# wuxiaolang/Cube_SLAM_wu

Hardware: AMD Instinct MI355X
Metric: frames/sec detect_cuboid (higher is better)
Workload: dtype f64

## Files before the change

cube_slam_wu_amd/capi.py:

```python
from __future__ import annotations

import os as _os
_os.environ.setdefault("GPU_MAX_HW_QUEUES", "8")
import ctypes as C
import os

import numpy as np

_HERE = os.path.dirname(os.path.abspath(__file__))
LIB_PATH = os.path.join(_HERE, "libcubeslam_hip.so")


class CsDetectParams(C.Structure):
    _fields_ = [
        ("consider_config_1", C.c_int), ("consider_config_2", C.c_int),
        ("whether_sample_cam_roll_pitch", C.c_int), ("whether_sample_bbox_height", C.c_int),
        ("max_cuboid_num", C.c_int), ("nominal_skew_ratio", C.c_double), ("max_cut_skew", C.c_double),
        ("yaw_range_deg", C.c_double), ("yaw_step_deg", C.c_double),
        ("vp12_edge_angle_thre", C.c_double), ("vp3_edge_angle_thre", C.c_double), ("shorted_edge_thre", C.c_double),
        ("weight_vp_angle", C.c_double), ("weight_skew_error", C.c_double),
        ("pre_merge_dist_thre", C.c_double), ("pre_merge_angle_thre", C.c_double), ("edge_length_threshold", C.c_double),
        ("host_threads", C.c_int),
    ]

# ... 21 lines not shown
    ]


class CsDetectTiming(C.Structure):
    _fields_ = [(n, C.c_double) for n in ("setup_host_ms", "h2d_ms", "vp_kernel_ms", "cand_kernel_ms", "compact_ms", "d2h_ms",
                                          "rank_host_ms", "finalize_ms", "total_ms")] + \
               [("n_jobs", C.c_longlong), ("n_slots", C.c_longlong), ("n_valid", C.c_longlong),
                ("cand_kernel_bytes", C.c_longlong), ("cand_kernel_launches", C.c_int), ("n_fallback_boxes", C.c_int), ("n_redo_frames", C.c_int),
                ("rank_kernel_ms", C.c_double), ("line_setup_ms", C.c_double), ("score_kernel_ms", C.c_double), ("score_kernel_bytes", C.c_longlong)]


DECLARED_SYMBOLS = [
    "cs_last_error", "cs_device_count", "cs_diag_build", "cs_detect_default_params", "cs_box_rois", "cs_cam_euler_zyx", "cs_detector_create",
    "cs_detector_destroy", "cs_detect_cuboids", "cs_batch_create", "cs_batch_max_boxes", "cs_batch_run", "cs_batch_submit", "cs_batch_collect",
    "cs_bgr_to_gray", "cs_edge_distance_maps", "cs_edge_distance_maps_multi", "cs_detect_cuboids_gray", "cs_batch_create_gray", "cs_batch_refill_gray", "cs_batch_refill_wait", "cs_batch_destroy", "cs_batch_last_timing", "cs_batch_debug_candidates", "cs_batch_debug_kept", "cs_batch_set_debug", "cs_batch_set_pipeline_chunks", "cs_detect_lines_gray", "cs_detect_lines_batch", "cs_detect_lines_last_timing", "cs_detect_lsd_gray", "cs_detect_lsd_batch", "cs_detect_lsd_last_timing",
    "cs_check_score_atan2", "cs_check_score_sample_index",
]

_lib = None


def lib():
    global _lib
    if _lib is None:
        if not os.path.exists(LIB_PATH):
            raise RuntimeError("libcubeslam_hip.so not built: run `python -c 'import __graft_entry__ as g; g.build()'`")
        try:
            import torch
        except ImportError:
            pass
        L = C.CDLL(LIB_PATH)
# ... 307 lines not shown
            if rc < 0:
                raise RuntimeError("cs_batch_debug_candidates failed (%d): %s" % (rc, last_error()))
        return rows, corners

    def debug_kept(self, frame, box, k=0):
        L = lib()
        n = L.cs_batch_debug_kept(self.h, frame, box, k, 0, None, None)
        if n < 0:
            raise RuntimeError("cs_batch_debug_kept failed (%d)" % n)
        ids = np.zeros(n, np.int32)
        sc = np.zeros(n)
        if n:
            L.cs_batch_debug_kept(self.h, frame, box, k, n, ids.ctypes.data_as(C.POINTER(C.c_int)), _dp(sc))
        return ids, sc

    def close(self):
        if self.h:
            lib().cs_batch_destroy(self.h)
            self.h = C.c_void_p()

    def __del__(self):
        try:
            self.close()
        except Exception:
            pass


class CsBaTiming(C.Structure):
    _fields_ = [(n, C.c_double) for n in ("errors_ms", "linearize_ms", "reduce_ms", "schur_ms", "factor_ms", "backsub_ms", "update_ms", "total_ms")] + \
               [("n_linearizations", C.c_longlong), ("n_solves", C.c_longlong), ("linearize_bytes", C.c_longlong), ("schur_entries", C.c_longlong), ("structure_ms", C.c_double)]
# ... 655 lines not shown
```

cube_slam_wu_amd/csrc/detect_host.cpp:

```cpp
#include <hip/hip_runtime.h>

#include <algorithm>
#include <atomic>
#include <condition_variable>
#include <memory>
#include <mutex>
#include <chrono>
#include <cmath>
#include <limits>
#include <cstdio>
#include <cstring>
#include <functional>
#include <numeric>
#include <string>
#include <thread>
#include <vector>

#include "../../include/cubeslam_hip.h"
#include "cs_hip_util.h"
#include "detect_hooks.h"
#include "detect_types.h"
#include "edge_types.h"

thread_local std::string g_cs_err;
// ... 369 lines not shown
  std::vector<int> rp_idx;
  std::vector<int> keep;
  std::vector<double> score;
  std::vector<double> corners;
};

struct PipeSlot {
  DevBuf<cs::JobDesc> jobs;
  DevBuf<unsigned char> tab_arena;
  PinBuf<unsigned char> h_tab_arena;
  bool merged_io = false;
  size_t o_jobs = 0, o_rec = 0, o_wc = 0, o_fb = 0, o_jv = 0, o_cb = 0, o_end = 0;
  DevBuf<long long> slot_prefix, job_cbase, c_slot, fb_slot;
  DevBuf<int> vp_prefix, top_x, flag, job_valid, c_flag, box_job0, box_njobs, win_count, fallback, fb_flag;
  DevBuf<double> bound3;
  DevBuf<int> ls_order, blk_info, ls_crowded;
  PinBuf<int> h_ls_order;
  DevBuf<double> mid_x, mid_y, ang, yaw, yaw_c, yaw_s, vp, bound, c_dist, c_angle, c_skew, fb_dist, fb_angle, fb_skew;
  DevBuf<cs::RankWinner> winners;
  DevBuf<cs_cuboid> records;
  PinBuf<cs_cuboid> h_records;
  struct RpRound { size_t j0 = 0, nj = 0, b0 = 0, nb = 0; long long slot_cap = 0; int vp_cap = 0; };
  std::vector<RpRound> rp_rounds;
  std::vector<int> rp_box_frame, rp_box_index;
  DevBuf<int> rp_trip_cnt;
  DevBuf<int> rp_cur_idx, rp_tab_count, rp_maps;
  DevBuf<long long> rp_last_slot, rp_box_base;
  DevBuf<unsigned long long> rp_pool_used;
  DevBuf<double> rp_raw_euler;
  PinBuf<int> h_rp_tab_count, h_rp_maps;
// ... 10 lines not shown
  PinBuf<double> h_yaw, h_yaw_c, h_yaw_s;
  PinBuf<long long> h_fb_src, h_fb_dst, h_fb_slot, h_win_slots;
  PinBuf<int> h_fb_cnt, h_fb_flag;
  PinBuf<double> h_fb_dist, h_fb_angle, h_fb_skew, h_win_corners;
  hipEvent_t done = nullptr, ev[13] = {};
  cs::DetectDeviceView view{};
  int f0 = 0, f1 = 0, vp_total = 0;
  size_t nj = 0, nb = 0;
  long long slot_total = 0;
  bool in_flight = false;
  bool counted_busy = false;
  void release() {
    jobs.release(); slot_prefix.release(); job_cbase.release(); c_slot.release(); fb_slot.release();
    vp_prefix.release(); top_x.release(); flag.release(); job_valid.release(); c_flag.release(); box_job0.release(); box_njobs.release(); win_count.release();
    fallback.release(); fb_flag.release(); mid_x.release(); mid_y.release(); ang.release(); yaw.release(); yaw_c.release(); yaw_s.release();
    vp.release(); bound.release(); bound3.release(); ls_order.release(); blk_info.release(); ls_crowded.release(); h_ls_order.release(); c_dist.release(); c_angle.release(); c_skew.release(); fb_dist.release(); fb_angle.release(); fb_skew.release();
    winners.release(); records.release(); h_records.release(); rp_trip_cnt.release(); rp_cur_idx.release(); rp_tab_count.release(); rp_maps.release(); rp_last_slot.release(); rp_box_base.release(); rp_pool_used.release(); rp_raw_euler.release(); h_rp_tab_count.release(); h_rp_maps.release(); h_rp_raw_euler.release(); h_rp_last_slot.release(); h_rp_box_base.release(); h_rp_pool_used.release(); h_jobs_in.release(); h_jobs_out.release(); h_slot_prefix.release(); h_job_cbase.release(); h_vp_prefix.release();
    h_top_x.release(); h_box_job0.release(); h_box_njobs.release(); h_win_count.release(); h_fallback.release(); h_job_valid.release(); h_yaw.release();
    h_yaw_c.release(); h_yaw_s.release();
    h_fb_src.release(); h_fb_dst.release(); h_fb_slot.release(); h_win_slots.release(); h_fb_cnt.release(); h_fb_flag.release(); h_fb_dist.release(); h_fb_angle.release();
    h_fb_skew.release(); h_win_corners.release();
    if (done) (void)hipEventDestroy(done);
    for (auto& e : ev) if (e) (void)hipEventDestroy(e);
    for (auto& e : rp_ev) if (e) (void)hipEventDestroy(e);
    rp_ev.clear();
    done = nullptr; for (auto& e : ev) e = nullptr;
  }
};

struct BatchRunState;
struct cs_batch {
// ... 3 lines not shown
  DevBuf<unsigned char> d_gray, d_cls;
  DevBuf<cs::EdgeRoi> d_edge_rois;
  DevBuf<unsigned char> d_gray2;
  hipStream_t copy_stream = nullptr;
  hipEvent_t ev_copied[2] = {nullptr, nullptr}, ev_edge_done[2] = {nullptr, nullptr};
  int gray_cur = 0, gray_w = 0, gray_h = 0, edge_n_rois = 0, edge_max_w = 1;
  long long edge_max_px = 1;
  bool gray_batch = false;
  int refill_q[2] = {-1, -1}, n_refill = 0;
  PinBuf<float> h_maps_stage;
  PipeSlot pipe[2];
  std::vector<int> job_base, box_base, top_base;
  std::vector<long long> line_base;
  bool force_no_pipeline = false;
  int pipe_chunks = 1;
  int n_frames = 0, max_boxes = 0;
  std::vector<FrameIn> frames;
  DevBuf<float> d_maps;
  DevBuf<double> d_invK, d_frame_lines;
  DevBuf<int> d_frame_line_ptr;
  bool device_setup = false;
  bool force_host_setup = false;
  DevBuf<cs::JobDesc> d_jobs;
  DevBuf<long long> d_slot_prefix, d_job_cbase, d_c_slot, d_win_slots;
  DevBuf<int> d_vp_prefix, d_top_x, d_flag, d_job_valid, d_c_flag;
  DevBuf<double> d_mid_x, d_mid_y, d_ang, d_yaw, d_yaw_c, d_yaw_s, d_vp, d_bound, d_dist, d_angle, d_skew, d_corners, d_c_dist, d_c_angle, d_c_skew, d_win_corners;
  DevBuf<cs::RpPose> d_rp;
  PinBuf<char> h_stage;
  PinBuf<long long> h_c_slot, h_job_cbase;
  PinBuf<int> h_c_flag, h_job_valid;
// ... 653 lines not shown
      for (int q = 0; q < NBK; q++) cnt[q + 1] += cnt[q];
      for (size_t j = 0; j < nj; j++) S.h_ls_order.p[cnt[bucket(S.h_jobs_in.p[j])]++] = (int)j;
    }
    if (vo > 0x7fffffffLL) { cs_set_error("too many yaw samples in one chunk"); return CS_ERR_CAPACITY; }
  }
  S.nb = nb;
  MARK(1, tq);
  MARK(2, tq);
  C.tm->setup_host_ms += now_ms() - t0;
  C.tm->n_jobs += (long long)nj; C.tm->n_slots += real_slots;
  const long long slot_total = S.slot_total;
  PENS(S.ls_order, nj); PENS(S.jobs, nj); PENS(S.slot_prefix, nj + 1); PENS(S.vp_prefix, nj + 1); PENS(S.job_valid, nj); PENS(S.job_cbase, nj + 1);
  PENS(S.mid_x, n_lines + 1); PENS(S.mid_y, n_lines + 1); PENS(S.ang, n_lines + 1); PENS(S.yaw, n_yaw + 1); PENS(S.yaw_c, n_yaw + 1); PENS(S.yaw_s, n_yaw + 1);
  PENS(S.top_x, n_top + 1); PENS(S.vp, 6 * (size_t)S.vp_total + 6); PENS(S.bound, 6 * (size_t)S.vp_total + 6); PENS(S.bound3, nj * (size_t)cs::vp3_table_doubles_per_job());
  PENS(S.blk_info, 2 * (size_t)(slot_total >> 8) + 4); PENS(S.ls_crowded, 2 * (nj + 1) + 2);
  PENS(S.c_slot, slot_total + 1); PENS(S.c_flag, slot_total + 1); PENS(S.c_dist, slot_total + 1);
  PENS(S.c_angle, slot_total + 1); PENS(S.c_skew, slot_total + 1); PENS(S.box_job0, nb + 1); PENS(S.box_njobs, nb + 1); PENS(S.win_count, nb + 1);
  PENS(S.fallback, nb + 1); PENS(S.winners, nb * KMAX + 1); PENS(S.records, nb * KMAX + 1); PENS(S.h_records, nb * KMAX + 1);
  PENS(S.h_win_count, nb + 1); PENS(S.h_fallback, nb + 1); PENS(S.h_job_valid, nj); PENS(S.h_job_cbase, nj + 1); PENS(S.h_jobs_out, nj);
  int* p_ls_order = S.ls_order.p; cs::JobDesc* p_jobs = S.jobs.p; long long* p_slot_prefix = S.slot_prefix.p; int* p_vp_prefix = S.vp_prefix.p;
  double *p_yaw = S.yaw.p, *p_yaw_c = S.yaw_c.p, *p_yaw_s = S.yaw_s.p;
  int *p_top_x = S.top_x.p, *p_box_job0 = S.box_job0.p, *p_box_njobs = S.box_njobs.p;
  cs_cuboid* p_records = S.records.p; int *p_win_count = S.win_count.p, *p_fallback = S.fallback.p, *p_job_valid = S.job_valid.p; long long* p_job_cbase = S.job_cbase.p;
  std::unique_lock<std::mutex> enqueue(d->streams->enqueue_mu, std::defer_lock);
  S.merged_io = nj <= 256;
  if (S.merged_io) {
    size_t need = 0;
    auto room = [&](size_t bytes) { const size_t at = need; need += (bytes + 255) & ~(size_t)255; return at; };
    const size_t o_ls = room(sizeof(int) * nj), o_sp = room(sizeof(long long) * (nj + 1)), o_vp = room(sizeof(int) * (nj + 1));
    const size_t o_y = room(8 * n_yaw), o_yc = room(8 * n_yaw), o_ys = room(8 * n_yaw), o_tx = room(sizeof(int) * n_top), o_b0 = room(sizeof(int) * nb), o_bn = room(sizeof(int) * nb);
// ... 17 lines not shown
  } else {
    cs::CopySegs cp{};
    cs::add_copy(cp, S.ls_order, S.h_ls_order, nj); cs::add_copy(cp, S.jobs, S.h_jobs_in, nj); cs::add_copy(cp, S.slot_prefix, S.h_slot_prefix, nj + 1);
    cs::add_copy(cp, S.vp_prefix, S.h_vp_prefix, nj + 1); cs::add_copy(cp, S.yaw, S.h_yaw, n_yaw); cs::add_copy(cp, S.yaw_c, S.h_yaw_c, n_yaw);
    cs::add_copy(cp, S.yaw_s, S.h_yaw_s, n_yaw); cs::add_copy(cp, S.top_x, S.h_top_x, n_top); cs::add_copy(cp, S.box_job0, S.h_box_job0, nb);
    cs::add_copy(cp, S.box_njobs, S.h_box_njobs, nb);
    if (!d->streams->own_streams) enqueue.lock();
    cs::launch_multi_copy(cp, st);
  }
  cs::DetectDeviceView& v = S.view;
  v = cs::DetectDeviceView{};
  v.jobs = p_jobs; v.n_jobs = (int)nj; v.slot_prefix = p_slot_prefix; v.vp_prefix = p_vp_prefix; v.maps = b->d_maps.p;
  v.mid_x = S.mid_x.p; v.mid_y = S.mid_y.p; v.line_angle = S.ang.p; v.yaw = p_yaw; v.yaw_cos = p_yaw_c; v.yaw_sin = p_yaw_s; v.top_x = p_top_x;
  v.rp = b->d_rp.p; v.invK = b->d_invK.p; v.vp = S.vp.p; v.bound = S.bound.p; v.bound3 = S.bound3.p; v.job_valid = p_job_valid;
  v.job_cbase = p_job_cbase; v.c_slot = S.c_slot.p; v.c_flag = S.c_flag.p; v.c_dist = S.c_dist.p; v.c_angle = S.c_angle.p; v.c_skew = S.c_skew.p;
  hipStream_t stB = nullptr, stC = nullptr;
  sweep_side_streams(d, &stB, &stC);
  if (stB != st) {
    CS_HIP_TRY(hipEventRecord(S.ev[7], st));
    CS_HIP_TRY(hipStreamWaitEvent(stB, S.ev[7], 0));
  }
  CS_HIP_TRY(hipEventRecord(S.ev[8], stB));
  v.blk_info = S.blk_info.p;
  CS_HIP_TRY(hipMemsetAsync(S.blk_info.p, 0, sizeof(int), stB));
  cs::launch_candidate_compact(v, C.sp, stB);
  CS_HIP_TRY(hipEventRecord(S.ev[9], stB));
  CS_HIP_TRY(hipEventRecord(S.ev[10], stB));
  CS_HIP_TRY(hipEventRecord(S.ev[0], st));
  cs::launch_line_setup_listed(p_jobs, (int)nj, b->d_frame_lines.p, b->d_frame_line_ptr.p, S.mid_x.p, S.mid_y.p, S.ang.p, P.pre_merge_dist_thre, P.pre_merge_angle_thre, P.edge_length_threshold, st, p_ls_order,
                               stC, S.ev[0], S.ev[12], S.ls_crowded.p);
  CS_HIP_TRY(hipEventRecord(S.ev[1], st));
  cs::launch_vp_support_only(v, C.sp, S.vp_total, st, 1);
  CS_HIP_TRY(hipEventRecord(S.ev[2], st));
  if (stB != st) CS_HIP_TRY(hipStreamWaitEvent(st, S.ev[10], 0));
  CS_HIP_TRY(hipEventRecord(S.ev[4], st));
  cs::launch_score(v, C.sp, slot_total, slot_total, st);
  CS_HIP_TRY(hipEventRecord(S.ev[5], st));
  cs::RankView rv{};
  rv.box_job0 = p_box_job0; rv.box_njobs = p_box_njobs; rv.n_boxes = (int)nb; rv.winners = S.winners.p; rv.win_count = p_win_count; rv.fallback = p_fallback;
  cs::RankParams rkp{P.weight_vp_angle, P.weight_skew_error, P.nominal_skew_ratio, P.max_cut_skew, KMAX, C.sp.short_sq_bound};
  cs::launch_rank(v, rv, rkp, st, 0, false);
  cs::launch_records(v, rv, KMAX, p_records, st, nullptr, rkp.short_sq_bound);
  CS_HIP_TRY(hipEventRecord(S.ev[6], st));
  CS_HIP_TRY(hipGetLastError());
  if (S.merged_io) {
    CS_HIP_TRY(hipMemcpyAsync(S.h_tab_arena.p + S.o_jobs, S.tab_arena.p + S.o_jobs, S.o_end - S.o_jobs, hipMemcpyDeviceToHost, st));
  } else {
    cs::CopySegs cp{};
    cs::add_copy(cp, S.h_records, S.records, nb * KMAX); cs::add_copy(cp, S.h_win_count, S.win_count, nb); cs::add_copy(cp, S.h_fallback, S.fallback, nb);
// ... 580 lines not shown
  CS_GUARD_BEGIN
  return batch_run_impl(d, b, out, out_counts, false);
  CS_GUARD_END("cs_batch_run")
}
extern "C" int cs_batch_submit(cs_detector* d, cs_batch* b, cs_cuboid* out, int* out_counts) {
  CS_GUARD_BEGIN
  return batch_run_impl(d, b, out, out_counts, true);
  CS_GUARD_END("cs_batch_submit")
}
extern "C" int cs_batch_collect(cs_detector* d, cs_batch* b) {
  CS_GUARD_BEGIN
  if (!d || !b || b->det != d) return CS_ERR_INVALID_ARG;
  return batch_collect_impl(d, b);
  CS_GUARD_END("cs_batch_collect")
}
static void batch_drop_run_state(cs_batch* b) { delete b->run_state; b->run_state = nullptr; }
static int batch_collect_impl(cs_detector* d, cs_batch* b) {
  if (!b->run_state) return CS_OK;
  std::unique_ptr<BatchRunState> rs(b->run_state);
  b->run_state = nullptr;
  if (!rs->deferred) return CS_OK;
  CS_HIP_TRY(hipSetDevice(d->device));
  int rc = rs->rp_lean ? rp_finish(rs->C, b->pipe[0]) : pipe_finish(rs->C, b->pipe[0], rs->cam_rp);
  if (rc) return rc;
  rs->tm.total_ms = now_ms() - rs->t_begin;
  b->timing = rs->tm;
  b->ran = true;
  if (g_prof && (++g_runs % 8) == 0) {
    const char* nm[11] = {"jobs+samples", "prefix+pack", "box table", "alloc+enqueue", "gpu wait", "tie lists", "records", "tie wait", "tie rank", "tie corners", "tie records"};
    fprintf(stderr, "[detect] host ms/run:");
    for (int k = 0; k < 11; k++) { fprintf(stderr, " %s %.3f", nm[k], g_mark[k] / 8); g_mark[k] = 0; }
    fprintf(stderr, " | pre %.3f total %.3f\n", g_mark[11] / 8, rs->tm.total_ms); g_mark[11] = 0;
  }
  return CS_OK;
}
static int batch_run_impl(cs_detector* d, cs_batch* b, cs_cuboid* out, int* out_counts, bool defer) {
  if (!d || !b || b->det != d || !out || !out_counts) return CS_ERR_INVALID_ARG;
  if (b->run_state) { cs_set_error("cs_batch_submit: the previous submit of this batch has not been collected"); return CS_ERR_INVALID_ARG; }
  CS_HIP_TRY(hipSetDevice(d->device));
  { const int rcf = batch_flush_refill(d, b); if (rcf) return rcf; }
  std::unique_ptr<BatchRunState> rs_owner(new BatchRunState());
  BatchRunState* rs = rs_owner.get();
  const cs_detect_params& P = d->prm;
  const bool sample_rp = P.whether_sample_cam_roll_pitch != 0;
  const int NF = b->n_frames, MB = b->max_boxes, KMAX = P.max_cuboid_num;
  auto parallel_for = [d](int n, int , const std::function<void(int)>& fn) { d->pool->run(n, fn); };
  const int NT = d->n_threads;
  hipStream_t st = d->stream;
  cs_detect_timing& tm = rs->tm;
  double t_begin = now_ms();
  rs->t_begin = t_begin;

  std::fill(out_counts, out_counts + (size_t)NF * std::max(MB, 0), 0);
  b->results.clear();
  b->job_index.assign((size_t)NF * std::max(MB, 1) * 3, -1);

  cs::SweepParams sp;
  sp.vp12_thre_rad = P.vp12_edge_angle_thre / 180.0 * CS_PI;
  sp.vp3_thre_rad = P.vp3_edge_angle_thre / 180.0 * CS_PI;
  sp.short_thre = P.shorted_edge_thre;
  sp.short_sq_bound = cs::sqrt_lt_bound(P.shorted_edge_thre);
  sp.consider_config_1 = P.consider_config_1; sp.consider_config_2 = P.consider_config_2;

  double t0 = now_ms();
  std::vector<CamCache>& cam_raw = rs->cam_raw; cam_raw.resize(NF);
  std::vector<std::vector<CamCache>>& cam_rp = rs->cam_rp; cam_rp.resize(NF);
  std::vector<double> cur_yaw(NF);
  parallel_for(NF, NT, [&](int f) {
    const FrameIn& F = b->frames[f];
    make_cam(F.K, F.R, F.t, cam_raw[f]);
    cur_yaw[f] = cam_raw[f].cam_yaw;
    if (sample_rp) {
      std::vector<double> rs, ps;
      linespace<double>(cam_raw[f].euler[0] - 6.0 / 180.0 * CS_PI, cam_raw[f].euler[0] + 6.0 / 180.0 * CS_PI, 3.0 / 180.0 * CS_PI, rs);
      linespace<double>(cam_raw[f].euler[1] - 6.0 / 180.0 * CS_PI, cam_raw[f].euler[1] + 6.0 / 180.0 * CS_PI, 3.0 / 180.0 * CS_PI, ps);
      for (double r : rs)
        for (double p : ps) {
// ... 715 lines not shown
```

cube_slam_wu_amd/csrc/detect_kernels.hip:

```cpp
#include <hip/hip_runtime.h>
#include "cs_hip_util.h"

#include <cstdio>
#include <cstdlib>
#include <cstring>

#include "../../include/cubeslam_hip.h"
#include "detect_types.h"
#include "cs_atan2_lean.h"

namespace cs {

__device__ __forceinline__ int wave_uniform_i32(int x) { return __builtin_amdgcn_readfirstlane(x); }
__device__ __forceinline__ long long wave_uniform_i64(long long x) {
  const unsigned lo = (unsigned)__builtin_amdgcn_readfirstlane((int)(unsigned)(x & 0xffffffffll)), hi = (unsigned)__builtin_amdgcn_readfirstlane((int)(x >> 32));
  return (long long)(((unsigned long long)hi << 32) | lo);
}
__device__ __forceinline__ double wave_uniform_f64(double x) {
  int lo, hi;
  asm("v_readfirstlane_b32 %0, %1" : "=s"(lo) : "v"(__double2loint(x)));
  asm("v_readfirstlane_b32 %0, %1" : "=s"(hi) : "v"(__double2hiint(x)));
  return __hiloint2double(hi, lo);
}
template <typename T>
// ... 169 lines not shown
  }
  const double NaN = __builtin_nan("");
#pragma unroll
  for (int k = 0; k < K; k++) {
    const double ang_hi = R[k].have ? la[R[k].i_hi] : NaN, ang_lo = R[k].have ? la[R[k].i_lo] : NaN;
    out[2 * k] = swapped[k] ? ang_lo : ang_hi;
    out[2 * k + 1] = swapped[k] ? ang_hi : ang_lo;
  }
}

enum { VP3_RPCAP = 32 };

template <int MODE, bool UNIFORM>
__device__ __forceinline__ void vp_support_body(const DetectDeviceView& v, const SweepParams& sp, const JobDesc& jd, int j, long long e, bool on, VpChunk* ch) {
  int rp = 0, y = 0;
  if (on) {
    int local = (int)e - jd.vp_off;
    on = local < jd.RP * jd.Y;
    rp = local / jd.Y; y = local - rp * jd.Y;
  }
  double vpx[3] = {0, 0, 0}, vpy[3] = {0, 0, 0};
  if (on) {
    const RpPose* pose = v.rp + jd.rp_off + rp;
    double cy = v.yaw_cos[jd.yaw_off + y], sy = v.yaw_sin[jd.yaw_off + y];
    const double* A = pose->KinvR;
    double d[3][3] = {{cy, sy, 0.0}, {-sy, cy, 0.0}, {0.0, 0.0, 1.0}};
#pragma unroll
    for (int k = 0; k < 3; k++) {
      double h0 = (A[0] * d[k][0] + A[1] * d[k][1]) + A[2] * d[k][2];
      double h1 = (A[3] * d[k][0] + A[4] * d[k][1]) + A[5] * d[k][2];
      double h2 = (A[6] * d[k][0] + A[7] * d[k][1]) + A[8] * d[k][2];
      vpx[k] = h0 / h2;
      vpy[k] = h1 / h2;
    }
    if (MODE == 0) {
      double* vout = v.vp + 6 * e;
      vout[0] = vpx[0]; vout[1] = vpy[0]; vout[2] = vpx[1]; vout[3] = vpy[1]; vout[4] = vpx[2]; vout[5] = vpy[2];
    }
  }
  const double* mx = v.mid_x + jd.line_off;
  const double* my = v.mid_y + jd.line_off;
  const double* la = v.line_angle + jd.line_off;
  double b6[6];
  const double thre[3] = {sp.vp12_thre_rad, sp.vp12_thre_rad, sp.vp3_thre_rad};
  const bool swapped[3] = {false, true, true};
  vp_support_multi<(MODE == 0 ? 3 : 2), UNIFORM>(mx, my, la, jd.m, ch, vpx, vpy, thre, swapped, on, b6);
  if (!on) return;
  if (MODE == 1) { const double* t3 = v.bound3 + 2 * ((size_t)j * VP3_RPCAP + rp); b6[4] = t3[0]; b6[5] = t3[1]; }
  double* bout = v.bound + 6 * e;
#pragma unroll
  for (int q = 0; q < 6; q++) bout[q] = b6[q];
}

template <int MODE>
__global__ __launch_bounds__(256) void vp_support_kernel(DetectDeviceView v, SweepParams sp, int vp_total) {
  long long e = xcd_virtual_block() * blockDim.x + threadIdx.x;
  const bool on = e < vp_total;
  const int j = find_job_wave<int>(v.vp_prefix, v.n_jobs, on ? (int)e : vp_total - 1);
  const int ju = wave_uniform_i32(j);
  __shared__ VpChunk chunk[4];
  if (__all(j == ju)) vp_support_body<MODE, true>(v, sp, v.jobs[ju], ju, e, on, &chunk[threadIdx.x >> 6]);
  else vp_support_body<MODE, false>(v, sp, v.jobs[j], j, e, on, nullptr);
}
// ... 75 lines not shown
  unsigned long long valid = __ballot(flag != 0);
  if (valid) {
    int lane = threadIdx.x & 63;
    int j0 = __shfl(j, __ffsll((long long)valid) - 1);
    unsigned long long same = __ballot(flag != 0 && j == j0);
    if (same == valid) {
      if (lane == __ffsll((long long)valid) - 1) atomicAdd(&v.job_valid[j0], __popcll(valid));
    } else if (flag != 0) {
      atomicAdd(&v.job_valid[j], 1);
    }
  }
}

enum { COMPACT_PER = 16 };
enum { CC_TRIP = 4096 };
__global__ __launch_bounds__(256) void candidate_compact_kernel(DetectDeviceView v, SweepParams sp) {
  const int j = blockIdx.x;
  if (j >= v.n_jobs) return;
  __shared__ unsigned char s_flag[CC_TRIP];
  __shared__ int wsum[4];
  const int tid = threadIdx.x, lane = tid & 63, wid = tid >> 6;
  int jd_Y, jd_T, jd_rp_off, jd_yaw_off, jd_vp_off, jd_top_off, n_vp;
  BoxGeomD gd;
  {
    const JobDesc& jd = v.jobs[j];
    jd_Y = jd.Y; jd_T = jd.T; jd_rp_off = jd.rp_off; jd_yaw_off = jd.yaw_off; jd_vp_off = jd.vp_off; jd_top_off = jd.top_off;
    n_vp = jd.RP * jd.Y;
    const BoxGeomD g = box_geom_d(jd.g);
    gd = BoxGeomD{g.left, wave_uniform_f64(g.top), g.right, wave_uniform_f64(g.down),
                  wave_uniform_f64(g.el), wave_uniform_f64(g.et), wave_uniform_f64(g.er), wave_uniform_f64(g.eb)};
  }
  int* out_valid = v.job_valid + j;
  long long* out_cbase = v.job_cbase + j;
  asm volatile("" : "+v"(out_valid), "+v"(out_cbase));
  for (int e = tid; e < n_vp; e += 256) {
    const int rp = e / jd_Y, y = e - rp * jd_Y;
    const RpPose* pose = v.rp + jd_rp_off + rp;
    const double cy = v.yaw_cos[jd_yaw_off + y], sy = v.yaw_sin[jd_yaw_off + y];
    const double* A = pose->KinvR;
    const double d[3][3] = {{cy, sy, 0.0}, {-sy, cy, 0.0}, {0.0, 0.0, 1.0}};
    double* vout = v.vp + 6 * (long long)(jd_vp_off + e);
#pragma unroll
    for (int k = 0; k < 3; k++) {
      const double h0 = (A[0] * d[k][0] + A[1] * d[k][1]) + A[2] * d[k][2];
      const double h1 = (A[3] * d[k][0] + A[4] * d[k][1]) + A[5] * d[k][2];
      const double h2 = (A[6] * d[k][0] + A[7] * d[k][1]) + A[8] * d[k][2];
      vout[2 * k] = h0 / h2;
      vout[2 * k + 1] = h1 / h2;
    }
// ... 38 lines not shown
#pragma unroll
    for (int w = 0; w < 4; w++) { const int x = wsum[w]; if (w < wid) woff += x; total += x; }
    long long pos0 = run + woff;
    const long long sl0 = base + 2ll * r0 + wid * (64 * COMPACT_PER) + lane;
#pragma unroll
    for (int q = 0; q < COMPACT_PER; q++) {
      const unsigned long long bal = __ballot(f[q] != 0);
      if (f[q] != 0) {
        const long long pos = pos0 + __popcll(bal & below);
        v.c_slot[pos] = sl0 + q * 64;
        v.c_flag[pos] = f[q] | (j << CAND_JOB_SHIFT);
      }
      pos0 += __popcll(bal);
    }
    run += total;
    __syncthreads();
  }
  const int n_valid = (int)(run - base);
  if (tid == 0) { *out_valid = n_valid; *out_cbase = base; }
  const int nblk = (n_valid + 255) >> 8;
  if (nblk > 0) {
    __shared__ int s_at;
    if (tid == 0) s_at = atomicAdd(&v.blk_info[0], nblk);
    __syncthreads();
    const int at = s_at, b0 = (int)(base >> 8);
    for (int k = tid; k < nblk; k += 256) {
      const int left = n_valid - 256 * k;
      v.blk_info[2 + 2 * (long long)(at + k)] = b0 + k;
      v.blk_info[3 + 2 * (long long)(at + k)] = left > 256 ? 256 : left;
    }
  }
}

__device__ __forceinline__ int slot_corners(const DetectDeviceView& v, const JobDesc& jd, long long slot, double short_sq_bound, V2 c[8]) {
// ... 1208 lines not shown
    o.camera_pitch_delta = pose.pitch - raw_euler[3 * jd.frame + 1];
  }
  out[e] = o;
}

static inline unsigned grid8(long long n, int bs) {
  long long nb = (n + bs - 1) / bs;
  nb = (nb + 7) / 8 * 8;
  return (unsigned)(nb < 8 ? 8 : nb);
}

void launch_vp_support(const DetectDeviceView& v, const SweepParams& sp, int vp_total, hipStream_t st) {
  if (vp_total <= 0) return;
  vp_support_kernel<0><<<dim3(grid8(vp_total, 256)), dim3(256), 0, st>>>(v, sp, vp_total);
}
void launch_vp_support_only(const DetectDeviceView& v, const SweepParams& sp, int vp_total, hipStream_t st, int rp_max) {
  if (skip_kernel("vp_support")) return;
  if (vp_total <= 0) return;
  const int stride = (rp_max >= 1 && rp_max <= (int)VP3_RPCAP) ? rp_max : (int)VP3_RPCAP;
  hipLaunchKernelGGL(vp3_support_kernel, dim3((unsigned)(((long long)v.n_jobs * stride + 63) / 64)), dim3(64), 0, st, v, sp, stride);
  vp_support_kernel<1><<<dim3(grid8(vp_total, 256)), dim3(256), 0, st>>>(v, sp, vp_total);
}
int vp3_table_doubles_per_job() { return 2 * VP3_RPCAP; }
void launch_vp_points(const DetectDeviceView& v, int vp_total, hipStream_t st) {
  if (vp_total <= 0) return;
  hipLaunchKernelGGL(vp_points_kernel, dim3((vp_total + 255) / 256), dim3(256), 0, st, v, vp_total);
}
void launch_candidates(const DetectDeviceView& v, const SweepParams& sp, long long slot_total, hipStream_t st) {
  if (skip_kernel("candidate")) return;
  if (slot_total <= 0) return;
  hipLaunchKernelGGL(candidate_kernel, dim3(grid8(slot_total, 256)), dim3(256), 0, st, v, sp, slot_total);
}
void launch_candidate_compact(const DetectDeviceView& v, const SweepParams& sp, hipStream_t st) {
  if (skip_kernel("candidate")) return;
  if (v.n_jobs <= 0) return;
  hipLaunchKernelGGL(candidate_compact_kernel, dim3(v.n_jobs), dim3(256), 0, st, v, sp);
// ... 374 lines not shown
```

cube_slam_wu_amd/csrc/detect_types.h:

```cpp
#pragma once
#include <hip/hip_runtime.h>

#include <cstdint>

#include "../../include/cubeslam_hip.h"
#include "cs_geom.h"

namespace cs {

struct JobDesc {
  BoxGeom g;
  int map_w;
  int m;
  int Y;
  int T;
  int RP;
  int down_expand;
  int line_off;
  int yaw_off;
  int top_off;
  int rp_off;
  int vp_off;
  int frame, box, hid;
  long long map_off;
// ... 19 lines not shown
  const double* mid_x; const double* mid_y; const double* line_angle;
  const double* yaw; const double* yaw_cos; const double* yaw_sin;
  const int* top_x;
  const RpPose* rp;
  const double* invK;
  double* vp;
  double* bound;
  double* bound3;
  int* flag;
  int* job_valid;
  long long* job_cbase;
  long long* c_slot;
  double* c_dist; double* c_angle; double* c_skew;
  int* c_flag;
  int* blk_info;
};

struct RankParams {
  double w_angle;
  double w_skew;
  double nominal_skew;
  double max_cut_skew;
  int kmax;
  double short_sq_bound;
};
enum { RANK_KMAX = 8 };

struct RankWinner {
  long long slot;
  double normalized_error, dist_err, angle_err;
// ... 18 lines not shown
  long long* box_base;
  double* p_dist; double* p_angle; double* p_skew; int* p_flag; long long* p_slot;
};

struct RpCarryView {
  int n_frames, NT, YCAP;
  const int* prev_box_of_frame;
  const long long* prev_last_slot;
  const JobDesc* prev_jobs; const int* prev_box_job0; const int* prev_box_njobs;
  const int* job0_of_frame; const int* njobs_of_frame;
  const int* tab_count;
  int* cur_idx;
};

void launch_vp_support(const DetectDeviceView& v, const SweepParams& sp, int vp_total, hipStream_t st);
void launch_vp_support_only(const DetectDeviceView& v, const SweepParams& sp, int vp_total, hipStream_t st, int rp_max = 0);
void launch_vp_points(const DetectDeviceView& v, int vp_total, hipStream_t st);
int vp3_table_doubles_per_job();
void launch_candidates(const DetectDeviceView& v, const SweepParams& sp, long long slot_total, hipStream_t st);
void launch_candidate_compact(const DetectDeviceView& v, const SweepParams& sp, hipStream_t st);
void launch_scan_compact(const DetectDeviceView& v, hipStream_t st);
void launch_scan_compact_trips(const DetectDeviceView& v, int* cnt, int max_trips, hipStream_t st);
void launch_score(const DetectDeviceView& v, const SweepParams& sp, long long n_valid_bound, long long slot_total, hipStream_t st);
void launch_score_atan2_check(const double* y, const double* x, int n, double* out, int* accepted, hipStream_t st);
void launch_score_sample_index_check(const double* sy, const double* sx, const int* map_w, const double* a, const double* b, int n, int* index, double* probe, hipStream_t st);
void launch_gather_corners(const DetectDeviceView& v, const SweepParams& sp, const long long* slots, int n, double* out, hipStream_t st);
void launch_rank(const DetectDeviceView& v, const RankView& rv, const RankParams& rp, hipStream_t st, long long max_slots_per_box = 0, bool with_corners = true);
void launch_records(const DetectDeviceView& v, const RankView& rv, int kmax, cs_cuboid* out, hipStream_t st, const double* raw_euler = nullptr, double rebuild_short_sq_bound = -1.0);
void launch_rp_carry(const RpCarryView& c, JobDesc* jobs, hipStream_t st);
void launch_rp_save_fallback(const DetectDeviceView& v, const RpSaveView& s, hipStream_t st);
void launch_line_setup(JobDesc* jobs, int n_jobs, const double* frame_lines, const int* frame_line_ptr, double* mid_x, double* mid_y, double* line_angle,
// ... 9 lines not shown
```

include/cubeslam_hip.h:

```cpp
#ifndef CUBESLAM_HIP_H
#define CUBESLAM_HIP_H

#include <stddef.h>
#include <stdint.h>

#ifdef __cplusplus
extern "C" {
#endif

typedef enum cs_status {
  CS_OK = 0,
  CS_ERR_INVALID_ARG = -1,
  CS_ERR_HIP = -2,
  CS_ERR_NO_DEVICE = -3,
  CS_ERR_CAPACITY = -4,
  CS_ERR_NOT_RUN = -5
} cs_status;

const char* cs_last_error(void);
int cs_device_count(void);
int cs_diag_build(void);


typedef struct cs_detect_params {
// ... 100 lines not shown
  double line_setup_ms;
  double score_kernel_ms;
  long long score_kernel_bytes;
} cs_detect_timing;
int cs_batch_last_timing(const cs_batch* b, cs_detect_timing* t);

int cs_batch_set_debug(cs_batch* b, int enable);

int cs_batch_set_pipeline_chunks(cs_batch* b, int n_chunks);

int cs_batch_debug_candidates(cs_batch* b, int frame, int box, int k, int cap, double* rows9, double* corners16);
int cs_batch_debug_kept(cs_batch* b, int frame, int box, int k, int cap, int* keep_ids, double* scores);

int cs_check_score_atan2(const double* y, const double* x, int n, double* out, int* accepted);
int cs_check_score_sample_index(const double* sy, const double* sx, const int* map_w, const double* a, const double* b, int n, int* index, double* probe);


typedef struct cs_ba cs_ba;

int cs_ba_create(int device, cs_ba** out);
void cs_ba_destroy(cs_ba* ba);
int cs_ba_set_vertices(cs_ba* ba, const double* cams7, const int* cam_fixed, int n_cams,
                       const double* cuboids10, const int* cub_fixed, int n_cuboids,
                       const double* points3, const int* pt_fixed, int n_points, int cuboids_first);
int cs_ba_set_estimates(cs_ba* ba, const double* cams7, const double* cuboids10, const double* points3);
int cs_ba_set_edges_proj(cs_ba* ba, int n, const int* point, const int* cam, const double* uv2,
                         const double* info4, const double* intr4, const double* huber);
int cs_ba_set_edges_proj_stereo(cs_ba* ba, int n, const int* point, const int* cam, const double* uvr3,
                                const double* info9, const double* intr5, const double* huber);
int cs_ba_set_edges_cuboid(cs_ba* ba, int n, const int* cam, const int* cuboid, const double* meas10, const double* info81);
// ... 125 lines not shown
```

Measured before the change: 580,700.

## Compute VP support bounds only for vanishing points with surviving candidates

The candidate compaction kernel now records a per-job bitmap of which (roll/pitch, yaw) vanishing-point entries have any valid candidate and writes a compacted list of used entries. A new vp_support_kernel mode reads that list and computes support bounds only for those entries, taking VP coordinates from the precomputed vp array. To allow this, the main stream now waits on the side-stream event before the VP support launch, which reorders cross-stream synchronisation. A check entry point is added to compare full against used-only bounds.

```diff
diff --git a/cube_slam_wu_amd/capi.py b/cube_slam_wu_amd/capi.py
--- a/cube_slam_wu_amd/capi.py
+++ b/cube_slam_wu_amd/capi.py
@@ -59,7 +59,7 @@
     "cs_last_error", "cs_device_count", "cs_diag_build", "cs_detect_default_params", "cs_box_rois", "cs_cam_euler_zyx", "cs_detector_create",
     "cs_detector_destroy", "cs_detect_cuboids", "cs_batch_create", "cs_batch_max_boxes", "cs_batch_run", "cs_batch_submit", "cs_batch_collect",
     "cs_bgr_to_gray", "cs_edge_distance_maps", "cs_edge_distance_maps_multi", "cs_detect_cuboids_gray", "cs_batch_create_gray", "cs_batch_refill_gray", "cs_batch_refill_wait", "cs_batch_destroy", "cs_batch_last_timing", "cs_batch_debug_candidates", "cs_batch_debug_kept", "cs_batch_set_debug", "cs_batch_set_pipeline_chunks", "cs_detect_lines_gray", "cs_detect_lines_batch", "cs_detect_lines_last_timing", "cs_detect_lsd_gray", "cs_detect_lsd_batch", "cs_detect_lsd_last_timing",
-    "cs_check_score_atan2", "cs_check_score_sample_index",
+    "cs_check_score_atan2", "cs_check_score_sample_index", "cs_check_vp_support_used",
 ]
 
 _lib = None
@@ -397,6 +397,25 @@
             L.cs_batch_debug_kept(self.h, frame, box, k, n, ids.ctypes.data_as(C.POINTER(C.c_int)), _dp(sc))
         return ids, sc
 
+    def check_vp_support_used(self, bitmap_cap=0):
+        L = lib()
+        dims = (C.c_longlong * 3)()
+        nul = [None] * 10
+        rc = L.cs_check_vp_support_used(self.det.h, self.h, int(bitmap_cap), dims, *nul)
+        if rc != 0:
+            raise RuntimeError("cs_check_vp_support_used failed (%d): %s" % (rc, last_error()))
+        nj, nvp, nsl = (int(x) for x in dims)
+        r = dict(bound_full=np.zeros((nvp, 6)), bound_used=np.zeros((nvp, 6)), vp_used=np.zeros(nvp, np.int32), vp_n_used=np.zeros(nj, np.int32),
+                 vp_prefix=np.zeros(nj + 1, np.int32), job_shape=np.zeros((nj, 4), np.int32), slot_prefix=np.zeros(nj + 1, np.int64),
+                 c_slot=np.zeros(nsl, np.int64), job_valid=np.zeros(nj, np.int32), job_cbase=np.zeros(nj, np.int64))
+        if nj:
+            lp = lambda a: a.ctypes.data_as(C.POINTER(C.c_longlong))
+            rc = L.cs_check_vp_support_used(self.det.h, self.h, int(bitmap_cap), dims, _dp(r["bound_full"]), _dp(r["bound_used"]), _ip(r["vp_used"]), _ip(r["vp_n_used"]),
+                                            _ip(r["vp_prefix"]), _ip(r["job_shape"]), lp(r["slot_prefix"]), lp(r["c_slot"]), _ip(r["job_valid"]), lp(r["job_cbase"]))
+            if rc != 0:
+                raise RuntimeError("cs_check_vp_support_used failed (%d): %s" % (rc, last_error()))
+        return r
+
     def close(self):
         if self.h:
             lib().cs_batch_destroy(self.h)
diff --git a/cube_slam_wu_amd/csrc/detect_host.cpp b/cube_slam_wu_amd/csrc/detect_host.cpp
--- a/cube_slam_wu_amd/csrc/detect_host.cpp
+++ b/cube_slam_wu_amd/csrc/detect_host.cpp
@@ -407,6 +407,7 @@
   DevBuf<long long> slot_prefix, job_cbase, c_slot, fb_slot;
   DevBuf<int> vp_prefix, top_x, flag, job_valid, c_flag, box_job0, box_njobs, win_count, fallback, fb_flag;
   DevBuf<double> bound3;
+  DevBuf<int> vp_used, vp_n_used;
   DevBuf<int> ls_order, blk_info, ls_crowded;
   PinBuf<int> h_ls_order;
   DevBuf<double> mid_x, mid_y, ang, yaw, yaw_c, yaw_s, vp, bound, c_dist, c_angle, c_skew, fb_dist, fb_angle, fb_skew;
@@ -447,7 +448,7 @@
     jobs.release(); slot_prefix.release(); job_cbase.release(); c_slot.release(); fb_slot.release();
     vp_prefix.release(); top_x.release(); flag.release(); job_valid.release(); c_flag.release(); box_job0.release(); box_njobs.release(); win_count.release();
     fallback.release(); fb_flag.release(); mid_x.release(); mid_y.release(); ang.release(); yaw.release(); yaw_c.release(); yaw_s.release();
-    vp.release(); bound.release(); bound3.release(); ls_order.release(); blk_info.release(); ls_crowded.release(); h_ls_order.release(); c_dist.release(); c_angle.release(); c_skew.release(); fb_dist.release(); fb_angle.release(); fb_skew.release();
+    vp.release(); bound.release(); vp_used.release(); vp_n_used.release(); bound3.release(); ls_order.release(); blk_info.release(); ls_crowded.release(); h_ls_order.release(); c_dist.release(); c_angle.release(); c_skew.release(); fb_dist.release(); fb_angle.release(); fb_skew.release();
     winners.release(); records.release(); h_records.release(); rp_trip_cnt.release(); rp_cur_idx.release(); rp_tab_count.release(); rp_maps.release(); rp_last_slot.release(); rp_box_base.release(); rp_pool_used.release(); rp_raw_euler.release(); h_rp_tab_count.release(); h_rp_maps.release(); h_rp_raw_euler.release(); h_rp_last_slot.release(); h_rp_box_base.release(); h_rp_pool_used.release(); h_jobs_in.release(); h_jobs_out.release(); h_slot_prefix.release(); h_job_cbase.release(); h_vp_prefix.release();
     h_top_x.release(); h_box_job0.release(); h_box_njobs.release(); h_win_count.release(); h_fallback.release(); h_job_valid.release(); h_yaw.release();
     h_yaw_c.release(); h_yaw_s.release();
@@ -481,6 +482,7 @@
   std::vector<long long> line_base;
   bool force_no_pipeline = false;
   int pipe_chunks = 1;
+  bool lean_single = false;
   int n_frames = 0, max_boxes = 0;
   std::vector<FrameIn> frames;
   DevBuf<float> d_maps;
@@ -1164,6 +1166,7 @@
   PENS(S.mid_x, n_lines + 1); PENS(S.mid_y, n_lines + 1); PENS(S.ang, n_lines + 1); PENS(S.yaw, n_yaw + 1); PENS(S.yaw_c, n_yaw + 1); PENS(S.yaw_s, n_yaw + 1);
   PENS(S.top_x, n_top + 1); PENS(S.vp, 6 * (size_t)S.vp_total + 6); PENS(S.bound, 6 * (size_t)S.vp_total + 6); PENS(S.bound3, nj * (size_t)cs::vp3_table_doubles_per_job());
   PENS(S.blk_info, 2 * (size_t)(slot_total >> 8) + 4); PENS(S.ls_crowded, 2 * (nj + 1) + 2);
+  PENS(S.vp_used, (size_t)S.vp_total + 1); PENS(S.vp_n_used, nj);
   PENS(S.c_slot, slot_total + 1); PENS(S.c_flag, slot_total + 1); PENS(S.c_dist, slot_total + 1);
   PENS(S.c_angle, slot_total + 1); PENS(S.c_skew, slot_total + 1); PENS(S.box_job0, nb + 1); PENS(S.box_njobs, nb + 1); PENS(S.win_count, nb + 1);
   PENS(S.fallback, nb + 1); PENS(S.winners, nb * KMAX + 1); PENS(S.records, nb * KMAX + 1); PENS(S.h_records, nb * KMAX + 1);
@@ -1211,6 +1214,7 @@
   v.mid_x = S.mid_x.p; v.mid_y = S.mid_y.p; v.line_angle = S.ang.p; v.yaw = p_yaw; v.yaw_cos = p_yaw_c; v.yaw_sin = p_yaw_s; v.top_x = p_top_x;
   v.rp = b->d_rp.p; v.invK = b->d_invK.p; v.vp = S.vp.p; v.bound = S.bound.p; v.bound3 = S.bound3.p; v.job_valid = p_job_valid;
   v.job_cbase = p_job_cbase; v.c_slot = S.c_slot.p; v.c_flag = S.c_flag.p; v.c_dist = S.c_dist.p; v.c_angle = S.c_angle.p; v.c_skew = S.c_skew.p;
+  v.vp_used = S.vp_used.p; v.vp_n_used = S.vp_n_used.p;
   hipStream_t stB = nullptr, stC = nullptr;
   sweep_side_streams(d, &stB, &stC);
   if (stB != st) {
@@ -1226,10 +1230,10 @@
   CS_HIP_TRY(hipEventRecord(S.ev[0], st));
   cs::launch_line_setup_listed(p_jobs, (int)nj, b->d_frame_lines.p, b->d_frame_line_ptr.p, S.mid_x.p, S.mid_y.p, S.ang.p, P.pre_merge_dist_thre, P.pre_merge_angle_thre, P.edge_length_threshold, st, p_ls_order,
                                stC, S.ev[0], S.ev[12], S.ls_crowded.p);
+  if (stB != st) CS_HIP_TRY(hipStreamWaitEvent(st, S.ev[10], 0));
   CS_HIP_TRY(hipEventRecord(S.ev[1], st));
-  cs::launch_vp_support_only(v, C.sp, S.vp_total, st, 1);
+  cs::launch_vp_support_only(v, C.sp, S.vp_total, st, 1, true);
   CS_HIP_TRY(hipEventRecord(S.ev[2], st));
-  if (stB != st) CS_HIP_TRY(hipStreamWaitEvent(st, S.ev[10], 0));
   CS_HIP_TRY(hipEventRecord(S.ev[4], st));
   cs::launch_score(v, C.sp, slot_total, slot_total, st);
   CS_HIP_TRY(hipEventRecord(S.ev[5], st));
@@ -1840,6 +1844,65 @@
   return batch_collect_impl(d, b);
   CS_GUARD_END("cs_batch_collect")
 }
+static cs::SweepParams sweep_params_of(const cs_detect_params& P) {
+  cs::SweepParams sp;
+  sp.vp12_thre_rad = P.vp12_edge_angle_thre / 180.0 * CS_PI;
+  sp.vp3_thre_rad = P.vp3_edge_angle_thre / 180.0 * CS_PI;
+  sp.short_thre = P.shorted_edge_thre;
+  sp.short_sq_bound = cs::sqrt_lt_bound(P.shorted_edge_thre);
+  sp.consider_config_1 = P.consider_config_1; sp.consider_config_2 = P.consider_config_2;
+  return sp;
+}
+extern "C" int cs_check_vp_support_used(cs_detector* d, cs_batch* b, int bitmap_cap, long long dims[3], double* bound_full, double* bound_used, int* vp_used, int* vp_n_used,
+                                        int* vp_prefix, int* job_shape, long long* slot_prefix, long long* c_slot, int* job_valid, long long* job_cbase) {
+  CS_GUARD_BEGIN
+  if (!d || !b || b->det != d || !dims || bitmap_cap < 0) { cs_set_error("cs_check_vp_support_used: invalid argument"); return CS_ERR_INVALID_ARG; }
+  if (b->run_state || !b->lean_single) { cs_set_error("cs_check_vp_support_used: the batch's last sweep was not a collected one-chunk sweep of the lean path without roll/pitch sampling"); return CS_ERR_INVALID_ARG; }
+  PipeSlot& S = b->pipe[0];
+  const size_t nj = S.nj, nvp = (size_t)S.vp_total, nsl = (size_t)S.slot_total;
+  dims[0] = (long long)nj; dims[1] = (long long)nvp; dims[2] = (long long)nsl;
+  const bool any = bound_full || bound_used || vp_used || vp_n_used || vp_prefix || job_shape || slot_prefix || c_slot || job_valid || job_cbase;
+  if (!any || nj == 0) return CS_OK;
+  if (!(bound_full && bound_used && vp_used && vp_n_used && vp_prefix && job_shape && slot_prefix && c_slot && job_valid && job_cbase)) { cs_set_error("cs_check_vp_support_used: null array"); return CS_ERR_INVALID_ARG; }
+  CS_HIP_TRY(hipSetDevice(d->device));
+  hipStream_t st = d->stream;
+  CS_HIP_TRY(hipStreamSynchronize(st));
+  DevBuf<double> scratch;
+  std::vector<cs::JobDesc> jobs(nj);
+  int rc = scratch.ensure(2 * (6 * nvp + 6));
+  auto run = [&]() -> int {
+    const cs::SweepParams sp = sweep_params_of(d->prm);
+    cs::DetectDeviceView v = S.view;
+    v.vp_used_cap = bitmap_cap;
+    CS_HIP_TRY(hipMemsetAsync(v.blk_info, 0, sizeof(int), st));
+    CS_HIP_TRY(hipMemsetAsync(v.vp_used, 0xff, sizeof(int) * nvp, st));
+    CS_HIP_TRY(hipMemsetAsync(v.vp_n_used, 0xff, sizeof(int) * nj, st));
+    cs::launch_candidate_compact(v, sp, st);
+    v.bound = scratch.p;
+    cs::launch_vp_support_only(v, sp, (int)nvp, st, 1, false);
+    v.bound = scratch.p + 6 * nvp + 6;
+    CS_HIP_TRY(hipMemsetAsync(v.bound, 0xff, sizeof(double) * 6 * nvp, st));
+    cs::launch_vp_support_only(v, sp, (int)nvp, st, 1, true);
+    CS_HIP_TRY(hipGetLastError());
+    CS_HIP_TRY(hipStreamSynchronize(st));
+    CS_HIP_TRY(hipMemcpy(bound_full, scratch.p, sizeof(double) * 6 * nvp, hipMemcpyDeviceToHost));
+    CS_HIP_TRY(hipMemcpy(bound_used, scratch.p + 6 * nvp + 6, sizeof(double) * 6 * nvp, hipMemcpyDeviceToHost));
+    CS_HIP_TRY(hipMemcpy(vp_used, v.vp_used, sizeof(int) * nvp, hipMemcpyDeviceToHost));
+    CS_HIP_TRY(hipMemcpy(vp_n_used, v.vp_n_used, sizeof(int) * nj, hipMemcpyDeviceToHost));
+    CS_HIP_TRY(hipMemcpy(vp_prefix, v.vp_prefix, sizeof(int) * (nj + 1), hipMemcpyDeviceToHost));
+    CS_HIP_TRY(hipMemcpy(slot_prefix, v.slot_prefix, sizeof(long long) * (nj + 1), hipMemcpyDeviceToHost));
+    CS_HIP_TRY(hipMemcpy(c_slot, v.c_slot, sizeof(long long) * nsl, hipMemcpyDeviceToHost));
+    CS_HIP_TRY(hipMemcpy(job_valid, v.job_valid, sizeof(int) * nj, hipMemcpyDeviceToHost));
+    CS_HIP_TRY(hipMemcpy(job_cbase, v.job_cbase, sizeof(long long) * nj, hipMemcpyDeviceToHost));
+    CS_HIP_TRY(hipMemcpy(jobs.data(), v.jobs, sizeof(cs::JobDesc) * nj, hipMemcpyDeviceToHost));
+    for (size_t j = 0; j < nj; j++) { job_shape[4 * j] = jobs[j].Y; job_shape[4 * j + 1] = jobs[j].T; job_shape[4 * j + 2] = jobs[j].RP; job_shape[4 * j + 3] = jobs[j].m; }
+    return CS_OK;
+  };
+  if (rc == CS_OK) rc = run();
+  scratch.release();
+  return rc;
+  CS_GUARD_END("cs_check_vp_support_used")
+}
 static void batch_drop_run_state(cs_batch* b) { delete b->run_state; b->run_state = nullptr; }
 static int batch_collect_impl(cs_detector* d, cs_batch* b) {
   if (!b->run_state) return CS_OK;
@@ -1849,6 +1912,7 @@
   CS_HIP_TRY(hipSetDevice(d->device));
   int rc = rs->rp_lean ? rp_finish(rs->C, b->pipe[0]) : pipe_finish(rs->C, b->pipe[0], rs->cam_rp);
   if (rc) return rc;
+  b->lean_single = !rs->rp_lean;
   rs->tm.total_ms = now_ms() - rs->t_begin;
   b->timing = rs->tm;
   b->ran = true;
@@ -1878,15 +1942,11 @@
   rs->t_begin = t_begin;
 
   std::fill(out_counts, out_counts + (size_t)NF * std::max(MB, 0), 0);
+  b->lean_single = false;
   b->results.clear();
   b->job_index.assign((size_t)NF * std::max(MB, 1) * 3, -1);
 
-  cs::SweepParams sp;
-  sp.vp12_thre_rad = P.vp12_edge_angle_thre / 180.0 * CS_PI;
-  sp.vp3_thre_rad = P.vp3_edge_angle_thre / 180.0 * CS_PI;
-  sp.short_thre = P.shorted_edge_thre;
-  sp.short_sq_bound = cs::sqrt_lt_bound(P.shorted_edge_thre);
-  sp.consider_config_1 = P.consider_config_1; sp.consider_config_2 = P.consider_config_2;
+  const cs::SweepParams sp = sweep_params_of(P);
 
   double t0 = now_ms();
   std::vector<CamCache>& cam_raw = rs->cam_raw; cam_raw.resize(NF);
diff --git a/cube_slam_wu_amd/csrc/detect_kernels.hip b/cube_slam_wu_amd/csrc/detect_kernels.hip
--- a/cube_slam_wu_amd/csrc/detect_kernels.hip
+++ b/cube_slam_wu_amd/csrc/detect_kernels.hip
@@ -207,13 +207,24 @@
 template <int MODE, bool UNIFORM>
 __device__ __forceinline__ void vp_support_body(const DetectDeviceView& v, const SweepParams& sp, const JobDesc& jd, int j, long long e, bool on, VpChunk* ch) {
   int rp = 0, y = 0;
-  if (on) {
+  double vpx[3] = {0, 0, 0}, vpy[3] = {0, 0, 0};
+  if (MODE == 2) {
+    const int local = (int)e - jd.vp_off;
+    on = on && local < v.vp_n_used[j];
+    if (UNIFORM && !__any(on)) return;
+    if (on) {
+      const int entry = v.vp_used[jd.vp_off + local];
+      rp = jd.RP == 1 ? 0 : entry / jd.Y;
+      e = jd.vp_off + entry;
+      const double* vp = v.vp + 6 * e;
+      vpx[0] = vp[0]; vpy[0] = vp[1]; vpx[1] = vp[2]; vpy[1] = vp[3];
+    }
+  } else if (on) {
     int local = (int)e - jd.vp_off;
     on = local < jd.RP * jd.Y;
     rp = local / jd.Y; y = local - rp * jd.Y;
   }
-  double vpx[3] = {0, 0, 0}, vpy[3] = {0, 0, 0};
-  if (on) {
+  if (MODE != 2 && on) {
     const RpPose* pose = v.rp + jd.rp_off + rp;
     double cy = v.yaw_cos[jd.yaw_off + y], sy = v.yaw_sin[jd.yaw_off + y];
     const double* A = pose->KinvR;
@@ -239,7 +250,7 @@
   const bool swapped[3] = {false, true, true};
   vp_support_multi<(MODE == 0 ? 3 : 2), UNIFORM>(mx, my, la, jd.m, ch, vpx, vpy, thre, swapped, on, b6);
   if (!on) return;
-  if (MODE == 1) { const double* t3 = v.bound3 + 2 * ((size_t)j * VP3_RPCAP + rp); b6[4] = t3[0]; b6[5] = t3[1]; }
+  if (MODE != 0) { const double* t3 = v.bound3 + 2 * ((size_t)j * VP3_RPCAP + rp); b6[4] = t3[0]; b6[5] = t3[1]; }
   double* bout = v.bound + 6 * e;
 #pragma unroll
   for (int q = 0; q < 6; q++) bout[q] = b6[q];
@@ -345,12 +356,15 @@
 
 enum { COMPACT_PER = 16 };
 enum { CC_TRIP = 4096 };
+enum { CC_USED_BITS = 4096 };
 __global__ __launch_bounds__(256) void candidate_compact_kernel(DetectDeviceView v, SweepParams sp) {
   const int j = blockIdx.x;
   if (j >= v.n_jobs) return;
   __shared__ unsigned char s_flag[CC_TRIP];
   __shared__ int wsum[4];
+  __shared__ unsigned s_used[CC_USED_BITS / 32];
   const int tid = threadIdx.x, lane = tid & 63, wid = tid >> 6;
+  if (tid < CC_USED_BITS / 32) s_used[tid] = 0u;
   int jd_Y, jd_T, jd_rp_off, jd_yaw_off, jd_vp_off, jd_top_off, n_vp;
   BoxGeomD gd;
   {
@@ -364,6 +378,9 @@
   int* out_valid = v.job_valid + j;
   long long* out_cbase = v.job_cbase + j;
   asm volatile("" : "+v"(out_valid), "+v"(out_cbase));
+  unsigned long long out_n_used = (unsigned long long)(v.vp_n_used + j)
+                                  | (n_vp > ((v.vp_used_cap > 0 && v.vp_used_cap < (int)CC_USED_BITS) ? v.vp_used_cap : (int)CC_USED_BITS) ? 1ull : 0ull);
+  asm volatile("" : "+v"(out_n_used));
   for (int e = tid; e < n_vp; e += 256) {
     const int rp = e / jd_Y, y = e - rp * jd_Y;
     const RpPose* pose = v.rp + jd_rp_off + rp;
@@ -432,10 +449,38 @@
       pos0 += __popcll(bal);
     }
     run += total;
+    {
+      const unsigned r1 = min(r0 + (unsigned)(CC_TRIP / 2), half);
+      const unsigned e_lo = r0 / Tu, e_hi = (r1 - 1u) / Tu;
+#pragma unroll 1
+      for (unsigned e = e_lo + (unsigned)tid; e <= e_hi && e < (unsigned)CC_USED_BITS; e += 256u) {
+        const unsigned lo = max(e * Tu, r0) - r0, hi = min((e + 1u) * Tu, r1) - r0;
+        bool any = false;
+#pragma unroll 1
+        for (unsigned r = lo; r < hi && !any; r++) any = (s_flag[2u * r] | s_flag[2u * r + 1u]) != 0;
+        if (any) atomicOr(&s_used[e >> 5], 1u << (e & 31u));
+      }
+    }
     __syncthreads();
   }
   const int n_valid = (int)(run - base);
   if (tid == 0) { *out_valid = n_valid; *out_cbase = base; }
+  if (wid == 0) {
+    const int n_ent = v.jobs[j].RP * v.jobs[j].Y;
+    int* used = v.vp_used + v.jobs[j].vp_off;
+    int n_used = 0;
+    const bool track_used = (out_n_used & 1ull) == 0ull;
+    if (half > 0) {
+      for (int e0 = 0; e0 < n_ent; e0 += 64) {
+        const int e = e0 + lane;
+        const bool u = e < n_ent && (!track_used || ((s_used[e >> 5] >> (e & 31)) & 1u) != 0u);
+        const unsigned long long bal = __ballot(u);
+        if (u) used[n_used + __popcll(bal & below)] = e;
+        n_used += __popcll(bal);
+      }
+    }
+    if (lane == 0) *(int*)(out_n_used & ~1ull) = n_used;
+  }
   const int nblk = (n_valid + 255) >> 8;
   if (nblk > 0) {
     __shared__ int s_at;
@@ -1674,12 +1719,13 @@
   if (vp_total <= 0) return;
   vp_support_kernel<0><<<dim3(grid8(vp_total, 256)), dim3(256), 0, st>>>(v, sp, vp_total);
 }
-void launch_vp_support_only(const DetectDeviceView& v, const SweepParams& sp, int vp_total, hipStream_t st, int rp_max) {
+void launch_vp_support_only(const DetectDeviceView& v, const SweepParams& sp, int vp_total, hipStream_t st, int rp_max, bool used_only) {
   if (skip_kernel("vp_support")) return;
   if (vp_total <= 0) return;
   const int stride = (rp_max >= 1 && rp_max <= (int)VP3_RPCAP) ? rp_max : (int)VP3_RPCAP;
   hipLaunchKernelGGL(vp3_support_kernel, dim3((unsigned)(((long long)v.n_jobs * stride + 63) / 64)), dim3(64), 0, st, v, sp, stride);
-  vp_support_kernel<1><<<dim3(grid8(vp_total, 256)), dim3(256), 0, st>>>(v, sp, vp_total);
+  if (used_only) vp_support_kernel<2><<<dim3(grid8(vp_total, 256)), dim3(256), 0, st>>>(v, sp, vp_total);
+  else vp_support_kernel<1><<<dim3(grid8(vp_total, 256)), dim3(256), 0, st>>>(v, sp, vp_total);
 }
 int vp3_table_doubles_per_job() { return 2 * VP3_RPCAP; }
 void launch_vp_points(const DetectDeviceView& v, int vp_total, hipStream_t st) {
diff --git a/cube_slam_wu_amd/csrc/detect_types.h b/cube_slam_wu_amd/csrc/detect_types.h
--- a/cube_slam_wu_amd/csrc/detect_types.h
+++ b/cube_slam_wu_amd/csrc/detect_types.h
@@ -57,6 +57,9 @@
   double* c_dist; double* c_angle; double* c_skew;
   int* c_flag;
   int* blk_info;
+  int* vp_used;
+  int* vp_n_used;
+  int vp_used_cap;
 };
 
 struct RankParams {
@@ -105,7 +108,7 @@
 };
 
 void launch_vp_support(const DetectDeviceView& v, const SweepParams& sp, int vp_total, hipStream_t st);
-void launch_vp_support_only(const DetectDeviceView& v, const SweepParams& sp, int vp_total, hipStream_t st, int rp_max = 0);
+void launch_vp_support_only(const DetectDeviceView& v, const SweepParams& sp, int vp_total, hipStream_t st, int rp_max = 0, bool used_only = false);
 void launch_vp_points(const DetectDeviceView& v, int vp_total, hipStream_t st);
 int vp3_table_doubles_per_job();
 void launch_candidates(const DetectDeviceView& v, const SweepParams& sp, long long slot_total, hipStream_t st);
diff --git a/include/cubeslam_hip.h b/include/cubeslam_hip.h
--- a/include/cubeslam_hip.h
+++ b/include/cubeslam_hip.h
@@ -138,6 +138,8 @@
 
 int cs_check_score_atan2(const double* y, const double* x, int n, double* out, int* accepted);
 int cs_check_score_sample_index(const double* sy, const double* sx, const int* map_w, const double* a, const double* b, int n, int* index, double* probe);
+int cs_check_vp_support_used(cs_detector* d, cs_batch* b, int bitmap_cap, long long dims[3], double* bound_full, double* bound_used, int* vp_used, int* vp_n_used,
+                             int* vp_prefix, int* job_shape, long long* slot_prefix, long long* c_slot, int* job_valid, long long* job_cbase);
 
 
 typedef struct cs_ba cs_ba;
```

After: 582,400, median of 5. About the same (+0.3%).
